# sdoira/U96-SLAM

Hardware: AMD Instinct MI355X
Metric: Mpix-disparities/s (higher is better)
Workload: dtype u8

## Files before the change

### u96-slam_amd/csrc/sbm_api.hip

```cpp
#include <stdio.h>
#include <stdlib.h>
#include <string.h>

#include <algorithm>
#include <mutex>
#include <new>

#include "sbm_handle.h"

using namespace sbm;

enum BmStage { kBmPrefilter, kBmSad, kBmBorder, kBmLr, kBmSpeckle, kBmTotal, kBmStageCount };
enum BmMark { kBmBegin, kBmPrefiltered, kBmMatched, kBmChecked, kBmEnd, kBmMarkCount };
static const char* const kBmNames[] = {"prefilter", "sad", "border", "lrcheck", "speckle", "total"};
StageTable sbm::bm_stages() { return stage_table<kBmStageCount, 0>(kBmNames); }
static_assert(kBmMarkCount == sbm_handle::kMarks, "the ring holds one event per mark");

extern "C" {

void sbm_params_default(sbm_params* p, int num_disparities, int block_size) {
  if (!p) return;
  memset(p, 0, sizeof(*p));
  p->prefilter_type = SBM_PREFILTER_XSOBEL;
  p->prefilter_size = 9;
  p->prefilter_cap = 31;
  p->block_size = block_size > 0 ? block_size : 21;
  p->min_disparity = 0;
  p->num_disparities = num_disparities > 0 ? num_disparities : 64;
  p->texture_threshold = 10;
  p->uniqueness_ratio = 15;
  p->speckle_window_size = 0;
  p->speckle_range = 0;
  p->disp12_max_diff = -1;
}

int sbm_params_validate(const sbm_params* p, int width, int height) {
  if (!p) return SBM_ERR_NULL;
  if (width <= 0 || height <= 0) return SBM_ERR_SIZE;
  if (p->prefilter_type != SBM_PREFILTER_NORMALIZED_RESPONSE && p->prefilter_type != SBM_PREFILTER_XSOBEL)
    return SBM_ERR_PREFILTER_TYPE;
  if (p->prefilter_size < 5 || p->prefilter_size > 255 || p->prefilter_size % 2 == 0) return SBM_ERR_PREFILTER_SIZE;
  if (p->prefilter_cap < 1 || p->prefilter_cap > 63) return SBM_ERR_PREFILTER_CAP;
  if (p->block_size < 5 || p->block_size > 255 || p->block_size % 2 == 0 || p->block_size >= std::min(width, height))
    return SBM_ERR_BLOCK_SIZE;
  if (p->num_disparities <= 0 || p->num_disparities % 16 != 0) return SBM_ERR_NUM_DISPARITIES;
  if (p->texture_threshold < 0) return SBM_ERR_TEXTURE;
  if (p->uniqueness_ratio < 0) return SBM_ERR_UNIQUENESS;
  return SBM_OK;
}

const char* sbm_strerror(int code) {
  switch (code) {
    case SBM_OK: return "ok";
    case SBM_ERR_NULL: return "null argument";
    case SBM_ERR_SIZE: return "bad image size or stride (all the images must have the same size)";
    case SBM_ERR_PREFILTER_TYPE: return "preFilterType must be PREFILTER_NORMALIZED_RESPONSE or PREFILTER_XSOBEL";
    case SBM_ERR_PREFILTER_SIZE: return "preFilterSize must be odd and be within 5..255";
    case SBM_ERR_PREFILTER_CAP: return "preFilterCap must be within 1..63";
    case SBM_ERR_BLOCK_SIZE: return "SADWindowSize must be odd, be within 5..255 and be not larger than image width or height";
    case SBM_ERR_NUM_DISPARITIES: return "numDisparities must be positive and divisible by 16";
    case SBM_ERR_TEXTURE: return "texture threshold must be non-negative";
    case SBM_ERR_UNIQUENESS: return "uniqueness ratio must be non-negative";
    case SBM_ERR_NO_DEVICE: return "no usable HIP device (this library has no CPU backend)";
    case SBM_ERR_HIP: return "HIP runtime error (see sbm_last_hip_error)";
    case SBM_ERR_NOMEM: return "out of memory";
    case SBM_ERR_UNSUPPORTED: return "configuration outside this build's limits";
    case SBM_ERR_BATCH: return "batch count must be positive";
    case SBM_ERR_OCC_FULL: return "occupancy map full: points were counted as overflow, not stored (see sbm_occ_overflow)";
    case SBM_ERR_VWD_FULL: return "visual-word dictionary full: the call's new words did not fit and nothing was added (see sbm_vwd_overflow)";
    default: return "unknown status";
  }
}

int sbm_version(void) { return SBM_VERSION_MAJOR * 1000 + SBM_VERSION_MINOR; }

static void free_buffers(sbm_handle* h) {
  h->each_set([](auto& s) { release_all(s); });
  release_set(h->bm); release_set(h->fp); release_set(h->fq);
  free_staging(h);
  h->sg.have_last = false;
}

static std::mutex g_pool_mu;
static constexpr int kPool = 4;
static constexpr size_t kPoolScratch = (size_t)512 << 20;
static sbm_handle* g_pool[kPool];
static int g_pool_n = 0;

static size_t scratch_bytes(sbm_handle* h) {
  size_t n = h->pin_bytes;
  h->each_set([&](auto& s) { n += bytes_held(s); });
  return n;
}

static void reset_profile(sbm_handle* h, int enabled) {
  h->profiling = enabled;
  h->calls = h->ncall = 0;
  h->instr = false;
  h->each_clock([](StageClock& c, const StageTable&) { c.reset(); });
}

static void destroy_now(sbm_handle* h);

void sbm_trim(void) {
  std::lock_guard<std::mutex> lock(g_pool_mu);
  for (int i = 0; i < g_pool_n; i++) destroy_now(g_pool[i]);
  g_pool_n = 0;
}

int sbm_create(sbm_handle** out, const sbm_params* p, int device) {
  if (!out || !p) return SBM_ERR_NULL;
  *out = nullptr;
  int ndev = 0;
  if (hipGetDeviceCount(&ndev) != hipSuccess || ndev <= 0 || device < 0 || device >= ndev) return SBM_ERR_NO_DEVICE;
  {
    std::lock_guard<std::mutex> lock(g_pool_mu);
    for (int i = 0; i < g_pool_n; i++)
      if (g_pool[i]->device == device) {
        sbm_handle* h = g_pool[i];
        g_pool[i] = g_pool[--g_pool_n];
        h->p = *p;
        h->last_hip = 0;
        h->have_last = h->sg.have_last = false;
        reset_profile(h, 0);
        *out = h;
        return SBM_OK;
      }
  }
  sbm_handle* h = new (std::nothrow) sbm_handle();
  if (!h) return SBM_ERR_NOMEM;
  memset(h, 0, sizeof(*h));
  h->p = *p;
  h->device = device;
  DeviceScope dscope(device);
  if (dscope.enter() != hipSuccess) {
    delete h;
    return SBM_ERR_NO_DEVICE;
  }
  bool ok = hipStreamCreateWithFlags(&h->stream, hipStreamNonBlocking) == hipSuccess;
  if (!ok) {
    destroy_now(h);
    return SBM_ERR_HIP;
  }
  h->ev_ok = true;
  for (int r = 0; r < sbm_handle::kRing; r++)
    for (int i = 0; i < sbm_handle::kMarks; i++) h->ev_ok &= hipEventCreate(&h->ev[r][i]) == hipSuccess;
  *out = h;
  return SBM_OK;
}

static void sync_all_streams(sbm_handle* h) {
  if (h->stream) hipStreamSynchronize(h->stream);
  if (h->stream_in) hipStreamSynchronize(h->stream_in);
  if (h->stream_out) hipStreamSynchronize(h->stream_out);
}

void sbm_destroy(sbm_handle* h) {
  if (!h) return;
  DeviceScope dscope(h->device);
  dscope.enter();
  h->fq_pending_dst = nullptr;
  h->fq_waited = h->fq_submitted;
  sync_all_streams(h);
  {
    std::lock_guard<std::mutex> lock(g_pool_mu);
    if (g_pool_n < kPool) {
      if (scratch_bytes(h) > kPoolScratch) {
        free_buffers(h);
      }
      g_pool[g_pool_n++] = h;
      return;
    }
  }
  destroy_now(h);
}

static void destroy_now(sbm_handle* h) {
  DeviceScope dscope(h->device);
  dscope.enter();
  sync_all_streams(h);
  free_buffers(h);
  h->each_clock([](StageClock& c, const StageTable&) { c.release(); });
  for (int r = 0; r < sbm_handle::kRing; r++)
    for (int i = 0; i < sbm_handle::kMarks; i++)
      if (h->ev[r][i]) hipEventDestroy(h->ev[r][i]);
  for (int i = 0; i < sbm_handle::kChunks; i++) {
    if (h->ev_in[i]) hipEventDestroy(h->ev_in[i]);
    if (h->ev_done[i]) hipEventDestroy(h->ev_done[i]);
  }
  for (int k = 0; k < 4; k++) {
    if (h->ev_fq_in[k]) hipEventDestroy(h->ev_fq_in[k]);
    if (h->ev_fq_done[k]) hipEventDestroy(h->ev_fq_done[k]);
    if (h->ev_fq_out[k]) hipEventDestroy(h->ev_fq_out[k]);
  }
  if (h->stream_in) hipStreamDestroy(h->stream_in);
  if (h->stream_out) hipStreamDestroy(h->stream_out);
  if (h->stream) hipStreamDestroy(h->stream);
  delete h;
}

int sbm_set_params(sbm_handle* h, const sbm_params* p) {
  if (!h || !p) return SBM_ERR_NULL;
  h->p = *p;
  return SBM_OK;
}

int sbm_get_params(const sbm_handle* h, sbm_params* p) {
  if (!h || !p) return SBM_ERR_NULL;
  *p = h->p;
  return SBM_OK;
}

void* sbm_stream(sbm_handle* h) { return h ? (void*)h->stream : nullptr; }
int sbm_last_hip_error(const sbm_handle* h) { return h ? h->last_hip : 0; }

int sbm_synchronize(sbm_handle* h) {
  if (!h) return SBM_ERR_NULL;
  DeviceScope dscope(h->device);
  HIPCHK(h, dscope.enter());
  HIPCHK(h, hipStreamSynchronize(h->stream));
  while (h->fq_waited != h->fq_submitted) {
    const int st = sbm_wait_oldest(h);
    if (st != SBM_OK) return st;
  }
  return SBM_OK;
}

int sbm_set_profiling(sbm_handle* h, int enabled) {
  if (!h) return SBM_ERR_NULL;
  reset_profile(h, enabled);
  return SBM_OK;
}

}

static void valid_roi(const sbm_params& p, int W, int H, int reading, int roi[4]) {
  int full[4] = {0, 0, W, H};
  const int* r1 = (p.roi1[2] > 0 && p.roi1[3] > 0) ? p.roi1 : full;
  const int* r2 = (p.roi2[2] > 0 && p.roi2[3] > 0) ? p.roi2 : full;
  const int sw2 = p.block_size / 2, maxd = p.min_disparity + p.num_disparities - 1;
  const int xmin = std::max(r1[0], r2[0] + maxd) + sw2;
  const int xmax = std::min(r1[0] + r1[2], r2[0] + r2[2] - ((reading & kReadRoiMinusMinD) ? p.min_disparity : 0)) - sw2;
  const int ymin = std::max(r1[1], r2[1]) + sw2;
  const int ymax = std::min(r1[1] + r1[3], r2[1] + r2[3]) - sw2;
  if (xmax - xmin > 0 && ymax - ymin > 0) {
    roi[0] = xmin; roi[1] = ymin; roi[2] = xmax - xmin; roi[3] = ymax - ymin;
  } else {
    roi[0] = roi[1] = roi[2] = roi[3] = 0;
  }
}

int sbm::bm_plan_geom(const sbm_params& p, int n, int width, int height, BmPlan* pl) {
  const int st = sbm_params_validate(&p, width, height);
  if (st != SBM_OK) return st;
  if (n > 32767 || height > 65535) return SBM_ERR_UNSUPPORTED;
  if (p.num_disparities > 4096) return SBM_ERR_UNSUPPORTED;
  memset(pl, 0, sizeof(*pl));
  Geom& g = pl->g;
  g.W = width; g.H = height; g.n = n;
  g.nd = p.num_disparities; g.mindisp = p.min_disparity; g.wsz = p.block_size; g.w2 = p.block_size / 2;
  g.cap = p.prefilter_cap; g.tex = p.texture_threshold; g.uniq = p.uniqueness_ratio;
  g.filtered = (p.min_disparity - 1) * 16;
  g.lofs = std::max(g.nd - 1 + g.mindisp, 0);
  g.rofs = -std::min(g.nd - 1 + g.mindisp, 0);
  g.width1 = width - g.rofs - g.nd + 1;
  g.xend = std::min(g.width1, width - g.lofs);
  g.want_cost = p.disp12_max_diff >= 0;
  g.padl = ((g.nd + 64 + 63) / 64) * 64;
  g.pitch = ((g.padl + width + 128 + 63) / 64) * 64;
  g.plane = g.pitch * height;

  int roi[4];
  g.reading = env_switch("SBM_CV_READING", 0);
  valid_roi(p, width, height, g.reading, roi);
  g.row0 = std::max(roi[1], 0); g.row1 = std::min(roi[1] + roi[3], height);
  g.col0 = std::max(std::min(roi[0], width), 0); g.col1 = std::max(std::min(roi[0] + roi[2], width), 0);
  const bool range_fits = !(g.lofs >= width || g.rofs >= width || g.width1 < 1);
  pl->any_rows = range_fits && roi[2] > 0 && roi[3] > 0 && g.row1 > g.row0;
  if (!pl->any_rows) { g.row0 = g.row1 = 0; }
  pl->in_envelope = pl->any_rows && sad_fast_supported(g);
  return SBM_OK;
}

void sbm::bm_plan_launches(const sbm_params& p, bool inplace_ok, BmPlan* pl) {
  Geom& g = pl->g;
  pl->fast = pl->in_envelope && inplace_ok;
  if (pl->fast) {
    g.cost16 = 1;
    g.pfshift = sad_fast_pfshift(g);
    const int xhi = std::min(g.W - g.lofs - 1, g.W - g.rofs - g.nd);
    const int fa = g.w2, fb = xhi - g.w2 + 1;
    const bool borders_visible = g.want_cost || g.col0 < g.lofs + fa || g.col1 > g.lofs + fb;
    pl->border = borders_visible && sad_fast_borders_in_launch(g);
    pl->wide_borders = borders_visible && !pl->border;
    pl->sad = kSadFast;
    sad_fast_plan(pl);
    if (pl->wide_borders) { pl->wide_l[0] = 0; pl->wide_l[1] = pl->f.xc0; pl->wide_r[0] = pl->f.xc1; pl->wide_r[1] = g.xend; }
  } else if (pl->any_rows) {
    const bool wide = sad_wide_supported(g) && env_switch("SBM_WIDE", 1);
    pl->sad = wide ? kSadWide : kSadGeneric;
    snprintf(pl->kernel, sizeof(pl->kernel), "%s",
             !wide ? "sad_generic_kernel" : (pl->in_envelope ? "sad_wide_kernel [in-place accumulate unavailable]" : "sad_wide_kernel"));
  }
  pl->speckle = p.speckle_range >= 0 && p.speckle_window_size > 0;
  if (pl->speckle) {
    speckle_plan(g, p.speckle_window_size, p.speckle_range, &pl->spk);
    size_t part[4];
    SpeckleScratch::bytes(g.n, g.W, g.H, part);
    for (int i = 0; i < 4; i++) pl->spk_bytes[i] = (long long)part[i];
  }
}

extern "C" {

static int ensure_scratch(sbm_handle* h, int n, int W, int H, int pitch, bool need_cost, bool need_speckle, size_t ho_bytes,
                          size_t ho_flags) {
  auto& s = h->bm;
  const bool fits = n <= s.n && W == s.W && H == s.H && pitch == s.pitch && s.pf_l.p;
  if (!fits) {
    HIPCHK(h, hipStreamSynchronize(h->stream));
    release_set(s);
    const size_t npix = (size_t)n * W * H, pfbytes = (size_t)n * pitch * H + 4096;
    HIPCHK(h, s.pf_l.grow(pfbytes, h->stream));
    HIPCHK(h, s.pf_r.grow(pfbytes, h->stream));
    HIPCHK(h, s.disp_pre.grow(npix * sizeof(int16_t), h->stream));
    HIPCHK(h, hipMemsetAsync(s.pf_l.p, 0, pfbytes, h->stream));
    HIPCHK(h, hipMemsetAsync(s.pf_r.p, 0, pfbytes, h->stream));
    s.n = n; s.W = W; s.H = H; s.pitch = pitch;
  }
  const size_t npix = (size_t)s.n * W * H;
  if (need_cost) HIPCHK(h, s.cost.grow(npix * sizeof(int32_t), h->stream));
  HIPCHK(h, s.lr_keys.grow(lr_keys_bytes(s.n, W, H, need_cost), h->stream));
  if (need_speckle) HIPCHK(h, s.spk.ensure(s.n, W, H, h->stream));
  if (ho_bytes) {
    const bool fresh = ho_bytes > s.handoff.bytes;
    HIPCHK(h, s.handoff.grow(ho_bytes, h->stream));
    if (fresh || ho_flags != s.ho_flags || s.ho_epoch == 0xffffffffu) {
      HIPCHK(h, hipMemsetAsync(s.handoff.p, 0, ho_flags, h->stream));
      s.ho_flags = ho_flags;
      s.ho_epoch = 0;
    }
  }
  return SBM_OK;
}

static inline void mark(sbm_handle* h, BmMark i) {
  if (h->instr) hipEventRecord(h->ev[h->calls % sbm_handle::kRing][i], h->stream);
}

static void collect_profile(sbm_handle* h) {
  unsigned nrec = std::min<unsigned>(h->calls, sbm_handle::kRing), first = 0;
  if (h->profiling == 1 && h->calls > 0) { first = (h->calls - 1) % sbm_handle::kRing; nrec = 1; }
  static const BmStage kStage[kBmMarkCount - 1] = {kBmPrefilter, kBmSad, kBmLr, kBmSpeckle};
  float acc[kBmMarkCount - 1] = {}, tot = 0.f;
  for (unsigned r = first; r < first + nrec; r++) {
    for (int i = 0; i < kBmMarkCount - 1; i++) {
      float ms = 0.f;
      if (hipEventElapsedTime(&ms, h->ev[r][i], h->ev[r][i + 1]) == hipSuccess) acc[i] += ms;
    }
    float ms = 0.f;
    if (hipEventElapsedTime(&ms, h->ev[r][kBmBegin], h->ev[r][kBmEnd]) == hipSuccess) tot += ms;
  }
  const float inv = nrec ? 1.f / nrec : 0.f;
  for (int i = 0; i < kBmMarkCount - 1; i++) h->bm.clock.ms[kStage[i]] = acc[i] * inv;
  h->bm.clock.ms[kBmTotal] = tot * inv;
}

int sbm_compute_device(sbm_handle* h, int n, const void* d_left, const void* d_right, int width, int height,
                       void* d_disp, int sync) {
  if (!h || !d_left || !d_right || !d_disp) return SBM_ERR_NULL;
  if (n <= 0) return SBM_ERR_BATCH;
  const sbm_params& p = h->p;
  BmPlan pl;
  const int st = bm_plan_geom(p, n, width, height, &pl);
  if (st != SBM_OK) return st;
  DeviceScope dscope(h->device);
  HIPCHK(h, dscope.enter());
  bool inplace = false;
  if (pl.in_envelope) HIPCHK(h, mqsad_inplace_ok(h->stream, &inplace));
  bm_plan_launches(p, inplace, &pl);
  const Geom& g = pl.g;
  size_t ho_flags = 0;
  const size_t ho_bytes = sad_fast_handoff_bytes(pl, &ho_flags);
  const int st2 = ensure_scratch(h, n, width, height, g.pitch, g.want_cost, pl.speckle, ho_bytes, ho_flags);
  if (st2 != SBM_OK) return st2;
  h->last = g; h->have_last = true;
  h->bm.ho_links = 0;
  if (pl.any_rows) snprintf(h->last_kernel, sizeof(h->last_kernel), "%s", pl.kernel);

  const uint8_t* dl = (const uint8_t*)d_left;
  const uint8_t* dr = (const uint8_t*)d_right;
  uint8_t *pf_l = h->bm.pf_l.as<uint8_t>(), *pf_r = h->bm.pf_r.as<uint8_t>();
  int16_t* disp_pre = h->bm.disp_pre.as<int16_t>();
  int32_t* cost = h->bm.cost.as<int32_t>();
  int16_t* out = (int16_t*)d_disp;

  h->instr = h->profiling && h->ev_ok && (h->profiling != 3 || (h->ncall & 3u) == 0);
  mark(h, kBmBegin);
  if (pl.any_rows) {
    if (p.prefilter_type == SBM_PREFILTER_XSOBEL) {
      HIPCHK(h, launch_prefilter(dl, dr, pf_l, pf_r, g, h->stream));
    } else {
      HIPCHK(h, h->bm.vsum.grow((size_t)2 * h->bm.n * width * height * sizeof(uint16_t), h->stream));
      HIPCHK(h, launch_prefilter_norm(dl, dr, pf_l, pf_r, h->bm.vsum.as<uint16_t>(), g, p.prefilter_size, h->stream));
    }
  }
  mark(h, kBmPrefiltered);
  if (pl.sad == kSadFast) {
    h->bm.ho_slots = (size_t)(pl.f.nseg - 1) * g.n * pl.f.strips;
    HIPCHK(h, launch_sad_fast(pf_l, pf_r, disp_pre, cost, pl, ho_bytes ? h->bm.handoff.p : nullptr, ho_bytes ? ++h->bm.ho_epoch : 0u,
                              &h->bm.ho_links, h->stream));
    if (pl.wide_borders) {
      HIPCHK(h, launch_sad_wide(pf_l, pf_r, disp_pre, cost, g, pl.wide_l[0], pl.wide_l[1], h->stream));
      HIPCHK(h, launch_sad_wide(pf_l, pf_r, disp_pre, cost, g, pl.wide_r[0], pl.wide_r[1], h->stream));
    }
  } else if (pl.sad == kSadWide) {
    HIPCHK(h, launch_sad_wide(pf_l, pf_r, disp_pre, cost, g, 0, g.xend, h->stream));
  } else if (pl.sad == kSadGeneric) {
    HIPCHK(h, launch_sad_generic(pf_l, pf_r, disp_pre, cost, g, 0, g.xend, h->stream));
  }
  mark(h, kBmMatched);
  HIPCHK(h, launch_lrcheck(disp_pre, cost, out, h->bm.lr_keys.as<unsigned long long>(), g, p.disp12_max_diff, h->stream));
  mark(h, kBmChecked);
  if (pl.speckle) HIPCHK(h, launch_speckle(out, h->bm.spk, g, pl.spk, p.speckle_window_size, h->stream));
  mark(h, kBmEnd);
  if (h->instr) h->calls++;
  h->ncall++;
  if (sync || h->profiling == 1) HIPCHK(h, hipStreamSynchronize(h->stream));
  return SBM_OK;
}

int sbm_debug_plan(const sbm_params* p, int n, int width, int height, int inplace_ok, void* out, size_t out_bytes) {
  if (!p || !out) return SBM_ERR_NULL;
  if (out_bytes != sizeof(BmPlan)) return SBM_ERR_SIZE;
  if (n <= 0) return SBM_ERR_BATCH;
  BmPlan pl;
  const int st = bm_plan(*p, n, width, height, inplace_ok != 0, &pl);
  if (st == SBM_OK) memcpy(out, &pl, sizeof(pl));
  return st;
}

int sbm_rect_map_device(sbm_handle* h, const sbm_rect_cam* cam, int width, int height, void* d_map, int sync) {
  if (!h || !cam || !d_map) return SBM_ERR_NULL;
  if (width <= 0 || height <= 0 || width > 32767 || height > 32767) return SBM_ERR_SIZE;
  DeviceScope dscope(h->device);
  HIPCHK(h, dscope.enter());
  HIPCHK(h, launch_rect_map(*cam, width, height, (int16_t*)d_map, h->stream));
  if (sync) HIPCHK(h, hipStreamSynchronize(h->stream));
  return SBM_OK;
}

int sbm_rect_remap_device(sbm_handle* h, int n, const void* d_src, const void* d_map, int width, int height, void* d_dst,
                          int sync) {
  if (!h || !d_src || !d_map || !d_dst) return SBM_ERR_NULL;
  if (n <= 0) return SBM_ERR_BATCH;
  if (width <= 0 || height <= 0 || width > 32767 || height > 32767) return SBM_ERR_SIZE;
  if (((size_t)width * height + 1023) / 1024 > 65535) return SBM_ERR_UNSUPPORTED;
  DeviceScope dscope(h->device);
  HIPCHK(h, dscope.enter());
  HIPCHK(h, launch_rect_remap((const uint8_t*)d_src, (const int16_t*)d_map, (uint8_t*)d_dst, n, width, height, h->stream));
  if (sync) HIPCHK(h, hipStreamSynchronize(h->stream));
  return SBM_OK;
}

int sbm_prefilter_device(sbm_handle* h, int n, const void* d_src, int width, int height, int flavour, int cap,
                         void* d_dst, int sync) {
  if (!h || !d_src || !d_dst) return SBM_ERR_NULL;
  if (n <= 0) return SBM_ERR_BATCH;
  if (width <= 0 || height <= 0) return SBM_ERR_SIZE;
  if (flavour != SBM_PREFILTER_FLAVOUR_CV && flavour != SBM_PREFILTER_FLAVOUR_RTL) return SBM_ERR_PREFILTER_TYPE;
  if (flavour == SBM_PREFILTER_FLAVOUR_CV && (cap < 1 || cap > 63)) return SBM_ERR_PREFILTER_CAP;
  if (n > 65534 || height > 65535 * 4) return SBM_ERR_UNSUPPORTED;
  DeviceScope dscope(h->device);
  HIPCHK(h, dscope.enter());
  HIPCHK(h, launch_prefilter_dense((const uint8_t*)d_src, (uint8_t*)d_dst, n, width, height,
                                   flavour == SBM_PREFILTER_FLAVOUR_RTL, cap, h->stream));
  if (sync) HIPCHK(h, hipStreamSynchronize(h->stream));
  return SBM_OK;
}

int sbm_disparity_to_float_device(sbm_handle* h, int n, const void* d_disp, int width, int height, void* d_out, int sync) {
  if (!h || !d_disp || !d_out) return SBM_ERR_NULL;
  if (n <= 0) return SBM_ERR_BATCH;
  if (width <= 0 || height <= 0) return SBM_ERR_SIZE;
  DeviceScope dscope(h->device);
  HIPCHK(h, dscope.enter());
  HIPCHK(h, launch_disp_to_float((const int16_t*)d_disp, (float*)d_out, (size_t)n * width * height, h->stream));
  if (sync) HIPCHK(h, hipStreamSynchronize(h->stream));
  return SBM_OK;
}

int sbm_decimate_device(sbm_handle* h, int n, const void* d_disp, int width, int height, int scale, void* d_out, int sync) {
  if (!h || !d_disp || !d_out) return SBM_ERR_NULL;
  if (n <= 0) return SBM_ERR_BATCH;
  if (width <= 0 || height <= 0 || scale <= 0) return SBM_ERR_SIZE;
  DeviceScope dscope(h->device);
  HIPCHK(h, dscope.enter());
  HIPCHK(h, launch_decimate((const int16_t*)d_disp, (int16_t*)d_out, n, width, height, scale, h->stream));
  if (sync) HIPCHK(h, hipStreamSynchronize(h->stream));
  return SBM_OK;
}

int sbm_reproject_device(sbm_handle* h, int n, const void* d_disp, int width, int height, int scale,
                         const sbm_stereo_model* model, int apply_local, void* d_xyz, int sync) {
  if (!h || !d_disp || !d_xyz || !model) return SBM_ERR_NULL;
  if (n <= 0) return SBM_ERR_BATCH;
  if (width <= 0 || height <= 0 || scale <= 0) return SBM_ERR_SIZE;
  DeviceScope dscope(h->device);
  HIPCHK(h, dscope.enter());
  HIPCHK(h, launch_reproject((const int16_t*)d_disp, (float*)d_xyz, n, width, height, scale, *model, apply_local, h->stream));
  if (sync) HIPCHK(h, hipStreamSynchronize(h->stream));
  return SBM_OK;
}

int sbm_keypoints3d_device(sbm_handle* h, const void* d_disp, int width, int height, const void* d_kpts, int nk,
                           const sbm_stereo_model* model, float min_depth, float max_depth, void* d_xyz, int sync) {
  if (!h || !d_disp || !model || (nk > 0 && (!d_kpts || !d_xyz))) return SBM_ERR_NULL;
  if (width <= 0 || height <= 0 || nk < 0) return SBM_ERR_SIZE;
  DeviceScope dscope(h->device);
  HIPCHK(h, dscope.enter());
  HIPCHK(h, launch_keypoints3d((const int16_t*)d_disp, (const float*)d_kpts, (float*)d_xyz, width, height, nk, *model,
                               min_depth, max_depth, h->stream));
  if (sync) HIPCHK(h, hipStreamSynchronize(h->stream));
  return SBM_OK;
}

int sbm_get_profile(sbm_handle* h, const char* name, float* ms) {
  if (!h || !name || !ms) return SBM_ERR_NULL;
  DeviceScope dscope(h->device);
  HIPCHK(h, dscope.enter());
  HIPCHK(h, hipStreamSynchronize(h->stream));
  if (h->profiling && h->ev_ok) collect_profile(h);
  const float* t = nullptr;
  h->each_clock([&](StageClock& c, const StageTable& tab) {
    for (int i = 0; i < tab.nstage; i++)
      if (!strcmp(name, tab.names[i])) t = &c.ms[i];
  });
  if (!t) return SBM_ERR_UNSUPPORTED;
  *ms = *t;
  return SBM_OK;
}

int sbm_last_kernel_name(sbm_handle* h, char* dst, size_t dst_bytes) {
  if (!h || !dst || dst_bytes == 0) return SBM_ERR_NULL;
  snprintf(dst, dst_bytes, "%s", h->last_kernel);
  return SBM_OK;
}

int sbm_debug_fetch(sbm_handle* h, int which, void* dst, size_t dst_bytes) {
  if (!h || !dst) return SBM_ERR_NULL;
  if (which >= 4 && which <= 6) return sgbm_debug_fetch(h, which, dst, dst_bytes);
  if (!h->have_last) return SBM_ERR_UNSUPPORTED;
  const Geom& g = h->last;
  DeviceScope dscope(h->device);
  HIPCHK(h, dscope.enter());
  HIPCHK(h, hipStreamSynchronize(h->stream));
  const size_t npix = (size_t)g.n * g.W * g.H;
  if (which == 0 || which == 1) {
    if (dst_bytes < npix) return SBM_ERR_SIZE;
    const uint8_t* src = (which == 0 ? h->bm.pf_l : h->bm.pf_r).as<uint8_t>();
    HIPCHK(h, hipMemcpy2D(dst, g.W, src + g.padl, g.pitch, g.W, (size_t)g.n * g.H, hipMemcpyDeviceToHost));
    uint8_t* d = (uint8_t*)dst;
    for (size_t i = 0; i < npix; i++) d[i] = (uint8_t)((d[i] - kPfBias) >> g.pfshift);
    return SBM_OK;
  }
  if (which == 2) {
    if (!h->bm.cost.p) return SBM_ERR_UNSUPPORTED;
    if (dst_bytes < npix * sizeof(int32_t)) return SBM_ERR_SIZE;
    if (g.cost16) {
      uint16_t* tmp = (uint16_t*)malloc(npix * sizeof(uint16_t));
      if (!tmp) return SBM_ERR_NOMEM;
      hipError_t e = hipMemcpy(tmp, h->bm.cost.p, npix * sizeof(uint16_t), hipMemcpyDeviceToHost);
      if (e == hipSuccess)
        for (size_t i = 0; i < npix; i++) ((int32_t*)dst)[i] = tmp[i];
      free(tmp);
      HIPCHK(h, e);
      return SBM_OK;
    }
    HIPCHK(h, hipMemcpy(dst, h->bm.cost.p, npix * sizeof(int32_t), hipMemcpyDeviceToHost));
    return SBM_OK;
  }
  if (which == 3) {
    if (dst_bytes < npix * sizeof(int16_t)) return SBM_ERR_SIZE;
    HIPCHK(h, hipMemcpy(dst, h->bm.disp_pre.p, npix * sizeof(int16_t), hipMemcpyDeviceToHost));
    int16_t* d = (int16_t*)dst;
    for (int i = 0; i < g.n; i++)
      for (int y = 0; y < g.H; y++) {
        int16_t* row = d + ((size_t)i * g.H + y) * g.W;
        const bool live = y >= g.row0 && y < g.row1;
        for (int x = 0; x < g.W; x++)
          if (!live || x < g.lofs || x >= g.lofs + g.xend) row[x] = (int16_t)g.filtered;
      }
    return SBM_OK;
  }
  if (which == 7) {
    if (dst_bytes < 2 * sizeof(int32_t)) return SBM_ERR_SIZE;
    int32_t* d = (int32_t*)dst;
    d[0] = 0;
    d[1] = (int32_t)h->bm.ho_links;
    if (!h->bm.ho_links) return SBM_OK;
    const size_t slots = h->bm.ho_slots;
    uint32_t* tmp = (uint32_t*)malloc(slots * sizeof(uint32_t));
    if (!tmp) return SBM_ERR_NOMEM;
    const hipError_t e = hipMemcpy(tmp, h->bm.handoff.as<uint32_t>() + slots, slots * sizeof(uint32_t), hipMemcpyDeviceToHost);
    if (e == hipSuccess)
      for (size_t i = 0; i < slots; i++) d[0] += tmp[i] == h->bm.ho_epoch;
    free(tmp);
    HIPCHK(h, e);
    return SBM_OK;
  }
  return SBM_ERR_UNSUPPORTED;
}

}
```

### u96-slam_amd/csrc/sbm_sad_fast.hip

```cpp
#include <string.h>

#include "sbm_sad_fast_kernel.h"

namespace sbm {

__global__ void __launch_bounds__(256) mqsad_inplace_selftest_kernel(unsigned* bad) {
  unsigned long long st = (unsigned long long)(blockIdx.x * 256 + threadIdx.x) * 0x9E3779B97F4A7C15ull + 88172645463325252ull;
  auto rnd = [&]() { st ^= st << 13; st ^= st >> 7; st ^= st << 17; return st; };
  unsigned nbad = 0;
  for (int it = 0; it < 64; it++) {
    unsigned long long accA[4], accR[4], win[4];
    const unsigned pat = (unsigned)rnd() & ((it & 1) ? 0x00ffffffu : 0x000000ffu);
#pragma unroll
    for (int q = 0; q < 4; q++) { accA[q] = accR[q] = rnd() & 0x3fff3fff3fff3fffull; win[q] = rnd(); }
#pragma unroll
    for (int r = 0; r < 3; r++)
#pragma unroll
      for (int q = 0; q < 4; q++) {
        accR[q] = __builtin_amdgcn_mqsad_pk_u16_u8(win[(q + r) & 3], pat, accR[q]);
        asm volatile("v_mqsad_pk_u16_u8 %0, %1, %2, %0" : "+v"(accA[q]) : "v"(win[(q + r) & 3]), "v"(pat));
      }
#pragma unroll
    for (int q = 0; q < 4; q++) nbad += accA[q] != accR[q];
  }
  if (nbad) atomicAdd(bad, nbad);
  atomicAdd(bad + 1, 1u);
}

hipError_t mqsad_inplace_ok(hipStream_t s, bool* ok) {
  static const bool forced_off = env_switch("SBM_FAST_INPLACE", 1) == 0;
  static std::mutex mu;
  static signed char known[64];
  *ok = false;
  int dev = 0;
  hipError_t e = hipGetDevice(&dev);
  if (e != hipSuccess || forced_off || dev < 0 || dev >= 64) return e;
  std::lock_guard<std::mutex> lock(mu);
  if (!known[dev]) {
    unsigned* d = nullptr;
    if ((e = hipMalloc(&d, 8)) != hipSuccess) return e;
    bool pass = true;
    const unsigned grids[3] = {256u, 1024u, 2048u};
    for (int k = 0; k < 3 && pass && e == hipSuccess; k++) {
      unsigned h[2] = {1u, 0u};
      e = hipMemsetAsync(d, 0, 8, s);
      if (e == hipSuccess) {
        hipLaunchKernelGGL(mqsad_inplace_selftest_kernel, dim3(grids[k]), dim3(256), 0, s, d);
        e = hipGetLastError();
      }
      if (e == hipSuccess) e = hipMemcpyAsync(h, d, 8, hipMemcpyDeviceToHost, s);
      if (e == hipSuccess) e = hipStreamSynchronize(s);
      pass = h[0] == 0u && h[1] == grids[k] * 256u;
    }
    const hipError_t ef = hipFree(d);
    if (e == hipSuccess) e = ef;
    if (e != hipSuccess) return e;
    known[dev] = pass ? 1 : -1;
  }
  *ok = known[dev] > 0;
  return hipSuccess;
}

int sad_fast_pfshift(const Geom& g) {
  static const int env = env_switch("SBM_FAST_PFSHIFT", 2);
  if (env <= 0 || !sad_fast_supported(g)) return 0;
  const long maxs = (long)g.wsz * g.wsz * 2 * g.cap;
  const int sh = std::min(env, g.wsz <= 15 ? 2 : 1);
  const long f = 1L << sh;
  if (f * 2 * g.cap + 1 > 255) return 0;
  if (f * maxs + (f - 1) > 65535) return 0;
  if (2 * (f * (maxs * g.uniq / 100 + 1)) >= 65535) return 0;
  if ((long)g.tex * f > 0x3fffffff) return 0;
  return sh == (g.wsz <= 15 ? 2 : 1) ? sh : 0;
}

bool sad_fast_borders_in_launch(const Geom& g) { return g.nd <= 256; }

bool sad_fast_supported(const Geom& g) {
  if (g.wsz < 5 || g.wsz > 31) return false;
  if (g.nd > kFastNdMax) return false;
  const long maxs = (long)g.wsz * g.wsz * 2 * g.cap;
  if (maxs > 65534) return false;
  if (2 * (maxs * g.uniq / 100 + 1) >= 65535) return false;
  if (g.row0 < g.w2 || g.row1 > g.H - g.w2 || g.row1 <= g.row0) return false;
  if ((long)g.plane * 4 >= (1L << 31)) return false;
  const int xhi = std::min(g.W - g.lofs - 1, g.W - g.rofs - g.nd);
  if (xhi - g.w2 + 1 <= g.w2) return false;
  return true;
}

static hipError_t sad_fast_dispatch(BmPlan& pl, const FastArgs* a, hipStream_t s) {
  switch (pl.g.wsz) {
    case 15: return launch_nd<5, 3>(pl, a, s);
    case 21: return launch_nd<7, 3>(pl, a, s);
    default: return launch_sad_fast_pw1(pl, a, s);
  }
}

static int fast_handoff_mode() { return std::max(0, std::min(2, env_switch("SBM_FAST_HANDOFF", 1))); }

static int fast_slots(int nd) { return nd <= 64 ? 4096 : 3072; }

constexpr double kFirstRoundStep = 0.10, kFirstRoundSpan = 0.40;

static int fast_segment_order(int nseg, long per_seg, int slots, int nd, unsigned char* at) {
  for (int k = 0; k < 64; k++) at[k] = (unsigned char)k;
  if (fast_handoff_mode() != 1 || nd > 128) return nseg;
  const long D = (slots + per_seg - 1) / per_seg + 1;
  if (D >= nseg) return nseg;
  int base = 0;
  for (int r = 0; r < (int)D; r++)
    for (int p = r; p < nseg; p += (int)D) at[p] = (unsigned char)base++;
  return (int)D;
}

void sad_fast_plan(BmPlan* pl) {
  const Geom& g = pl->g;
  FastPlan& a = pl->f;
  const int xhi = std::min(g.W - g.lofs - 1, g.W - g.rofs - g.nd);
  a.xc0 = g.w2; a.xc1 = xhi - g.w2 + 1;
  const int pw = g.wsz % 3 == 0 ? 3 : 1;
  const int nv = 64 - (g.wsz - pw);
  const int cs3_env = env_switch("SBM_FAST_CS3", 1);
  const int ncols = a.xc1 - a.xc0;
  const int nv3 = 64 - (g.wsz / 3 - 1);
  int triples = 0;
  if (pw == 3 && cs3_env) {
    triples = ncols / (3 * nv3);
    if (ncols - triples * 3 * nv3 > 2 * nv) triples++;
  }
  a.strips3 = 3 * triples;
  const int rem = std::max(0, ncols - triples * 3 * nv3);
  const int strips = a.strips3 + (rem + nv - 1) / nv;
  const int rows = g.row1 - g.row0;
  const int round1 = g.nd <= 256 ? 1536 : (g.nd <= 384 ? 1024 : 768);
  constexpr double kSegC = 0.196;
  const int slots_i = g.nd <= 64 ? 4096 : (g.nd <= 128 ? 3072 : round1);
  int nseg = 1;
  {
    const double prime = 0.2 * (g.wsz - 1);
    const double slots = slots_i;
    nseg = (int)(std::sqrt(kSegC * slots * rows / ((double)strips * g.n * prime)) + 0.5);
    nseg = std::max(1, std::min(nseg, std::max(1, rows / g.wsz)));
  }
  constexpr int kSmallRows = 8;
  constexpr long kFill = 5000;
  const int maxseg = std::max(nseg, std::min(64, rows / kSmallRows));
  const long per_seg = (long)strips * g.n;
  if (per_seg * maxseg * (g.nd > 128 ? (g.nd + 127) / 128 : 1) < 1800) {
    nseg = std::max(nseg, (int)std::min<long>(maxseg, 1023 / per_seg));
  } else {
    const int nseg1 = nseg;
    while (per_seg * nseg < kFill && nseg < maxseg) nseg++;
    if (g.nd > 128 && per_seg * nseg > round1 && 2 * per_seg * nseg < 3 * round1) nseg = std::max(nseg1, (int)((long)round1 * 1450 / 1536 / per_seg));
  }
  nseg = std::min(nseg, 64);
  int ns = 0;
  a.segrow[0] = g.row0;
  if (nseg < 3) {
    const int seg = (rows + nseg - 1) / nseg;
    for (int y = g.row0; y < g.row1; y += seg) a.segrow[++ns] = std::min(y + seg, g.row1);
  } else {
    unsigned char at[64];
    const int stride = fast_segment_order(nseg, per_seg, slots_i, g.nd, at);
    const int first_round = stride - 1;
    int len[64];
    {
      const double step = first_round > 1 ? std::min(kFirstRoundStep, kFirstRoundSpan / (first_round - 1)) : 0.0;
      double wgt[64], sum = 0;
      for (int p = 0; p < nseg; p++) {
        wgt[p] = p < nseg - 3 ? 1.0 : (p == nseg - 3 ? 0.75 : (p == nseg - 2 ? 0.5 : 0.25));
        if (stride < nseg && p < first_round) wgt[p] = std::min(wgt[p], 1.0 - step * (first_round - 1 - p));
        sum += wgt[p];
      }
      const double unit = rows / sum;
      double acc = 0;
      int y0 = 0;
      for (int p = 0; p < nseg; p++) {
        acc += wgt[p] * unit;
        const int y1 = p == nseg - 1 ? rows : std::min(rows, (int)(acc + 0.5));
        len[p] = y1 - y0;
        y0 = y1;
      }
    }
    int np = 0;
    for (int p = 0; p < nseg; p++)
      if (len[p] > 0) len[np++] = len[p];
    fast_segment_order(np, per_seg, slots_i, g.nd, at);
    int seglen[64];
    for (int p = 0; p < np; p++) seglen[at[p]] = len[p];
    for (int k = 0; k < np; k++) a.segrow[k + 1] = a.segrow[k] + seglen[k];
    ns = np;
  }
  nseg = ns;
  a.strips = strips; a.nseg = nseg;
  {
    const long maxs = (long)g.wsz * g.wsz * 2 * g.cap;
    a.uniq_plain = 8 * ((maxs * g.uniq / 100 + 1) << g.pfshift) <= 65535;
  }
  a.split = (long)strips * nseg * g.n < 1024;
  sad_fast_dispatch(*pl, nullptr, nullptr);
}

static unsigned long long fast_handoff_links(const BmPlan& pl, unsigned char* at) {
  const FastPlan& f = pl.f;
  const int mode = fast_handoff_mode();
  const int stride = fast_segment_order(f.nseg, (long)f.strips * pl.g.n, fast_slots(pl.g.nd), pl.g.nd, at);
  if (mode == 0 || f.NWAVES != 1 || !f.exact || f.nseg < 2) return 0;
  unsigned long long links = 0;
  for (int p = mode == 2 ? 1 : stride; p < f.nseg; p++) links |= 1ull << at[p];
  return links;
}

constexpr size_t kHandoffMaxBytes = (size_t)1 << 30;
size_t sad_fast_handoff_bytes(const BmPlan& pl, size_t* flag_bytes) {
  unsigned char at[64];
  *flag_bytes = 0;
  if (!pl.fast || !fast_handoff_links(pl, at)) return 0;
  const size_t slots = (size_t)(pl.f.nseg - 1) * pl.g.n * pl.f.strips;
  const size_t fb = (2 * slots * sizeof(u32) + 255) & ~(size_t)255;
  const size_t bytes = fb + slots * ((size_t)(pl.f.NDW / 4) * 512 + 256);
  if (bytes > kHandoffMaxBytes) return 0;
  *flag_bytes = fb;
  return bytes;
}

hipError_t launch_sad_fast(const uint8_t* pf_l, const uint8_t* pf_r, int16_t* disp, int32_t* cost, BmPlan& pl, void* handoff,
                           unsigned epoch, long* links, hipStream_t s) {
  const Geom& g = pl.g;
  const FastPlan& f = pl.f;
  FastArgs a;
  a.pf_l = pf_l; a.pf_r = pf_r; a.disp = disp; a.cost = g.want_cost ? reinterpret_cast<uint16_t*>(cost) : nullptr;
  a.W = g.W; a.H = g.H; a.pitch = g.pitch; a.padl = g.padl; a.plane = g.plane;
  a.nd = g.nd; a.mindisp = g.mindisp; a.lofs = g.lofs; a.rofs = g.rofs; a.tex = g.tex << g.pfshift; a.uniq = g.uniq;
  a.filtered = g.filtered; a.capb = (g.cap << g.pfshift) + kPfBias; a.pfshift = g.pfshift;
  a.row0 = g.row0; a.row1 = g.row1;
  static_assert(sizeof(a.segrow) == sizeof(f.segrow), "");
  memcpy(a.segrow, f.segrow, sizeof(a.segrow));
  a.strips = f.strips; a.nseg = f.nseg; a.npairs = g.n; a.strips3 = f.strips3; a.uniq_plain = f.uniq_plain;
  a.xc0 = f.xc0; a.xc1 = f.xc1;
  a.bord = f.bord; a.bnw = f.bnw; a.bseg = f.bseg; a.nbseg = f.nbseg;
  a.ho_link = fast_handoff_links(pl, a.segat);
  if (!handoff) a.ho_link = 0;
  a.ho = static_cast<u32*>(handoff); a.ho_epoch = epoch;
  a.segbase = 0; a.grid = f.grid;
  const long per_seg = (long)f.strips * g.n;
  *links = (long)__builtin_popcountll(a.ho_link) * per_seg;
  if (fast_handoff_mode() != 2 || !a.ho_link) return sad_fast_dispatch(pl, &a, s);
  for (int k = 0; k < f.nseg; k++) {
    a.segbase = k;
    a.grid = (int)per_seg + (k == 0 ? f.bord * f.nbseg : 0);
    if (k == 1) a.bord = 0;
    const hipError_t e = sad_fast_dispatch(pl, &a, s);
    if (e != hipSuccess) return e;
  }
  return hipSuccess;
}

}
```

### u96-slam_amd/csrc/sbm_sad_fast_strip.h

```cpp
#pragma once
#include "sbm_sad_fast_core.h"

namespace sbm {

template <int NDW, int NWAVES, int NTERM, int PW, bool EXACT_ND, int CS>
__device__ __forceinline__ void sad_fast_strip_dma(const FastArgs& a, unsigned char* __restrict__ const b0c, unsigned char* __restrict__ const b1c,
                                                   unsigned char* __restrict__ const xl1c,
                                                   u32* __restrict__ const xkey,
                                                   const int cbase, const int segi, const int pair, const int strip) {
  using L = FastLds<NDW, NTERM, PW, CS>;
  using D = DmaLds<NDW, NWAVES, NTERM, PW, CS>;
  using P = HPlan<NTERM, PW>;
  typedef __attribute__((address_space(3))) void* lds_vptr;
  constexpr int NQ = NDW / 4;
  constexpr int NR = NDW / 2;
  constexpr int NSLOT = L::NSLOT;
  constexpr int NIT = NSLOT / 64;
  constexpr int WSZ = PW * NTERM, W2 = WSZ / 2;
  constexpr int KS = L::KS;
  constexpr int NV = 64 - KS * (NTERM - 1);
  constexpr int XCH = D::XCH, XS = L::XS;
  constexpr bool HANDOFF = FastHandoff<NDW, NWAVES, EXACT_ND>::ON;

  const int lane = threadIdx.x & 63;
  const int wv = NWAVES > 1 ? __builtin_amdgcn_readfirstlane(threadIdx.x >> 6) : 0;
  const int d0 = wv * NDW;
  const int ndl = EXACT_ND ? NDW : a.nd - d0;
  const int c = cbase + CS * lane;
  const int xc = c + W2;
  const bool produces = lane < NV && xc >= a.xc0 && xc < a.xc1;
  const int ys = a.segrow[segi];
  const int ye = a.segrow[segi + 1];
  const uint8_t* pl = a.pf_l + (size_t)pair * a.plane + a.padl + a.lofs + cbase;
  const uint8_t* pr = a.pf_r + (size_t)pair * a.plane + a.padl + a.rofs + cbase + d0;
  uint2* const xacc = reinterpret_cast<uint2*>(xkey + 2 * NWAVES * 64);
  const unsigned lane_u = (unsigned)lane;
  const __amdgpu_buffer_rsrc_t rs_l = __builtin_amdgcn_make_buffer_rsrc(const_cast<uint8_t*>(pl), 0, 0x7fffffff, 0x00020000);
  const __amdgpu_buffer_rsrc_t rs_r = __builtin_amdgcn_make_buffer_rsrc(const_cast<uint8_t*>(pr), 0, 0x7fffffff, 0x00020000);
  uint4* const b0 = reinterpret_cast<uint4*>(b0c);
  uint4* const b1 = reinterpret_cast<uint4*>(b1c);
  uint4* const xq0 = b0;
  uint4* const xq1 = reinterpret_cast<uint4*>(xl1c);
  typedef u32x4 __attribute__((may_alias)) u32x4a;
  auto xt_of = [](uint4* const xq) { return reinterpret_cast<u32*>(xq + (XCH / 2) * XS); };
  const u32 capw = (u32)a.capb * 0x01010101u;

  u64 VB[NQ];
  {
    const u32 unit = (lane_u / (unsigned)KS) % (unsigned)NTERM == 0u ? FastTag<WSZ>::tag_unit(a.pfshift) : 0u;
#pragma unroll
    for (int q = 0; q < NQ; q++) {
      const u32 tq = (u32)((2 * q) / (NR / FastTag<WSZ>::NGRP)) * unit;
      VB[q] = __builtin_bit_cast(u64, make_uint2(tq, tq));
    }
  }
  u32 Vt = 0;

  auto pat_of = [](uint4* const buf) { return reinterpret_cast<u32*>(reinterpret_cast<unsigned char*>(buf) + D::PAT_OFS); };
  auto stage = [&](const int y, uint4* const buf) {
    const int rowoff = __builtin_amdgcn_readfirstlane(y * a.pitch);
#pragma unroll
    for (int it = 0; it < NIT; it++)
      __builtin_amdgcn_raw_ptr_buffer_load_lds(rs_r, (lds_vptr)(reinterpret_cast<u32*>(buf) + 64 * it), 4, (int)lane_u, rowoff + 64 * it, 0, 0);
    __builtin_amdgcn_raw_ptr_buffer_load_lds(rs_l, (lds_vptr)pat_of(buf), 4, (int)(CS * lane_u), rowoff, 0, 0);
  };
  auto landed = [] {
    __builtin_amdgcn_s_waitcnt(0);
    __builtin_amdgcn_fence(__ATOMIC_ACQUIRE, "wavefront");
    __builtin_amdgcn_wave_barrier();
  };
  auto reads_done = [] {
    __builtin_amdgcn_s_waitcnt(0xc07f);
    __builtin_amdgcn_wave_barrier();
  };
  auto published = [] {
    __builtin_amdgcn_fence(__ATOMIC_RELEASE, "wavefront");
    __builtin_amdgcn_wave_barrier();
  };
  auto apply = [&](uint4* const buf, const bool leave) {
    constexpr u32 PMASK = PW == 3 ? 0x00ffffffu : 0x000000ffu;
    const u32 pat = pat_of(buf)[lane] & PMASK;
    const u32 tv = __builtin_amdgcn_sad_u8(pat | (capw & ~PMASK), capw, 0u);
    auto quad = [&](const int q, const u32 lo, const u32 hi) {
      const u64 win = ((u64)hi << 32) | lo;
      if (!leave) {
        asm("v_mqsad_pk_u16_u8 %0, %1, %2, %0" : "+v"(VB[q]) : "v"(win), "v"(pat));
      } else {
        const uint2 tt = __builtin_bit_cast(uint2, __builtin_amdgcn_mqsad_pk_u16_u8(win, pat, 0ull));
        uint2 vb = __builtin_bit_cast(uint2, VB[q]);
        vb.x -= tt.x;
        vb.y -= tt.y;
        asm("" : "+v"(vb.x), "+v"(vb.y));
        VB[q] = __builtin_bit_cast(u64, vb);
      }
    };
    {
      const u32* const win4 = reinterpret_cast<const u32*>(buf) + CS * lane;
      if constexpr (EXACT_ND) {
  #pragma unroll
        for (int q0 = 0; q0 < NQ; q0 += 16) {
          u32 lo[16], hi[16];
  #pragma unroll
          for (int qq = 0; qq < 16 && q0 + qq < NQ; qq++) { lo[qq] = win4[4 * (q0 + qq)]; hi[qq] = win4[4 * (q0 + qq) + 4]; }
  #pragma unroll
          for (int qq = 0; qq < 16 && q0 + qq < NQ; qq++) quad(q0 + qq, lo[qq], hi[qq]);
        }
      } else {
  #pragma unroll
        for (int g = 0; g < NQ / 4; g++) {
          if (16 * g < ndl) {
            u32 lo[4], hi[4];
  #pragma unroll
            for (int k = 0; k < 4; k++) { lo[k] = win4[4 * (4 * g + k)]; hi[k] = win4[4 * (4 * g + k) + 4]; }
  #pragma unroll
            for (int k = 0; k < 4; k++) quad(4 * g + k, lo[k], hi[k]);
          }
        }
      }
    }
    Vt = leave ? Vt - tv : Vt + tv;
  };

  const size_t ho_slots = HANDOFF ? (size_t)(a.nseg - 1) * a.npairs * a.strips : 0;
  const size_t ho_mine = HANDOFF ? ((size_t)segi * a.npairs + pair) * a.strips + strip : 0;
  auto ho_rsrc = [&](const size_t slot) {
    unsigned char* const p = reinterpret_cast<unsigned char*>(a.ho) + ((2 * ho_slots * sizeof(u32) + 255) & ~(size_t)255) + slot * FastHandoff<NDW, NWAVES, EXACT_ND>::SLOT_B;
    return __builtin_amdgcn_make_buffer_rsrc(p, 0, FastHandoff<NDW, NWAVES, EXACT_ND>::SLOT_B, 0x00020000);
  };
  bool take = false;
  if constexpr (HANDOFF) {
    if ((a.ho_link >> segi) & 1) {
      const size_t from = ho_mine - (size_t)a.npairs * a.strips;
      take = __builtin_amdgcn_readfirstlane(__hip_atomic_load(a.ho + from, __ATOMIC_RELAXED, __HIP_MEMORY_SCOPE_AGENT)) == a.ho_epoch;
      if (take) {
        __builtin_amdgcn_fence(__ATOMIC_ACQUIRE, "agent");
        const __amdgpu_buffer_rsrc_t rs_h = ho_rsrc(from);
#pragma unroll
        for (int q = 0; q < NQ; q++) VB[q] = __builtin_bit_cast(u64, __builtin_amdgcn_raw_buffer_load_b64(rs_h, (int)(8 * lane_u), 512 * q, kHandoffAux));
        Vt = __builtin_amdgcn_raw_buffer_load_b32(rs_h, (int)(4 * lane_u), 512 * NQ, kHandoffAux);
        if (lane == 0) a.ho[ho_slots + from] = a.ho_epoch;
        stage(ys + W2, b0);
      }
    }
  }
  if (!take) {
    stage(ys - W2, b0);
    for (int i = 0; i < 2 * W2; i += 2) {
      landed();
      stage(ys - W2 + i + 1, b1);
      apply(b0, false);
      landed();
      stage(ys - W2 + i + 2, b0);
      apply(b1, false);
    }
  }
  const __amdgpu_buffer_rsrc_t rs_d = __builtin_amdgcn_make_buffer_rsrc(a.disp + (size_t)pair * a.W * a.H, 0, 0x7fffffff, 0x00020000);
  const __amdgpu_buffer_rsrc_t rs_c = __builtin_amdgcn_make_buffer_rsrc(a.cost + (size_t)pair * a.W * a.H, 0, 0x7fffffff, 0x00020000);
  const int ocol_u = __builtin_amdgcn_readfirstlane(2 * (a.lofs + cbase + W2));
  u32 res_prev = 0xffff0000u;
  auto flush = [&](const int yrow) {
    if (produces && (NWAVES == 1 || (yrow % NWAVES) == wv)) {
      const int orow_prev = __builtin_amdgcn_readfirstlane(2 * yrow * a.W) + ocol_u;
      u32 l3 = CS * lane_u;
      asm volatile("" : "+v"(l3));
      const int ocol = (int)(2 * l3);
      if (a.cost) __builtin_amdgcn_raw_buffer_store_b16((short)(res_prev >> 16), rs_c, ocol, orow_prev, 0);
      __builtin_amdgcn_raw_buffer_store_b16((short)res_prev, rs_d, ocol, orow_prev, 0);
    }
  };
  for (int y = ys; y < ye; y++) {
    landed();
    if (y > ys) {
      flush(y - 1);
      apply(b1, true);
    }
    reads_done();
    stage(y - W2, b1);
    apply(b0, false);

    __builtin_amdgcn_s_setprio(kFastPrioExchange);
    u32 S[NR];
    unsigned long long tex_ok = 0;
    u32 lx = lane_u;
    asm volatile("" : "+v"(lx));
    auto add4 = [](u32 (&acc)[4], const uint4 r) { acc[0] += r.x; acc[1] += r.y; acc[2] += r.z; acc[3] += r.w; };
#pragma unroll
    for (int q0 = 0; q0 < NQ; q0 += XCH) {
      const bool tex_now = q0 == 0;
      if (!EXACT_ND && 4 * q0 >= ndl) {
#pragma unroll
        for (int j = 2 * q0; j < 2 * (q0 + XCH); j++) S[j] = 0xffffffffu;
        continue;
      }
      u32 A[XCH / 2][4];
      u32 tA = Vt;
#pragma unroll
      for (int e = 0; e < XCH / 2; e++) {
        const uint2 v0 = __builtin_bit_cast(uint2, VB[q0 + 2 * e]), v1 = __builtin_bit_cast(uint2, VB[q0 + 2 * e + 1]);
        A[e][0] = v0.x; A[e][1] = v0.y; A[e][2] = v1.x; A[e][3] = v1.y;
        xq0[e * XS + lane] = make_uint4(v0.x, v0.y, v1.x, v1.y);
      }
      if (tex_now) xt_of(xq0)[lane] = Vt;
      published();
      if constexpr (P::S1 > 1) {
#pragma unroll
        for (int e = 0; e < XCH / 2; e++)
#pragma unroll
          for (int k = 1; k < P::S1; k++) add4(A[e], xq0[e * XS + lx + KS * k]);
        if (tex_now)
#pragma unroll
          for (int k = 1; k < P::S1; k++) tA += xt_of(xq0)[lx + KS * k];
        if constexpr (P::PUB1) {
#pragma unroll
          for (int e = 0; e < XCH / 2; e++) {
            if constexpr (HANDOFF) *reinterpret_cast<u32x4a*>(xq1 + e * XS + lane) = (u32x4){A[e][0], A[e][1], A[e][2], A[e][3]};
            else xq1[e * XS + lane] = make_uint4(A[e][0], A[e][1], A[e][2], A[e][3]);
          }
          if (tex_now) xt_of(xq1)[lane] = tA;
          published();
        }
      }
      {
        constexpr int OV = P::NTT * P::S1;
#pragma unroll
        for (int e = 0; e < XCH / 2; e++) {
#pragma unroll
          for (int t = 1; t < P::NTT; t++) {
            if constexpr (HANDOFF) {
              const u32x4 r = *reinterpret_cast<const u32x4a*>(xq1 + e * XS + lx + KS * P::S1 * t);
              add4(A[e], make_uint4(r.x, r.y, r.z, r.w));
            } else {
              add4(A[e], xq1[e * XS + lx + KS * P::S1 * t]);
            }
          }
#pragma unroll
          for (int v = (P::NTT > 0 ? 0 : 1); v < P::NVV; v++) add4(A[e], xq0[e * XS + lx + KS * (OV + v)]);
        }
        if (tex_now) {
#pragma unroll
          for (int t = 1; t < P::NTT; t++) tA += xt_of(xq1)[lx + KS * P::S1 * t];
#pragma unroll
          for (int v = (P::NTT > 0 ? 0 : 1); v < P::NVV; v++) tA += xt_of(xq0)[lx + KS * (OV + v)];
          tex_ok = __ballot((int)tA >= a.tex);
        }
      }
#pragma unroll
      for (int e = 0; e < XCH / 2; e++)
#pragma unroll
        for (int i = 0; i < 4; i++) S[2 * (q0 + 2 * e) + i] = A[e][i];
      __builtin_amdgcn_wave_barrier();
    }
    reads_done();
    stage(min(y + 1 + W2, a.H - 1), b0);
    __builtin_amdgcn_s_setprio(0);

    u32 best = fast_first_min<NR, WSZ>(S, a.pfshift);
    best += (u32)d0;
    const int par = y & 1, mpar = par * NWAVES * 64;
    if constexpr (NWAVES > 1) {
      xkey[mpar + wv * 64 + lane] = best;
      __syncthreads();
#pragma unroll
      for (int w = 0; w < NWAVES; w++) best = min(best, xkey[mpar + w * 64 + lane]);
    }
    const int minsad = (int)(best >> 16), mind = (int)(best & 0xffffu);

    u32 acc = 0, T = 0;
    if (a.uniq > 0) {
      T = fast_uniq_threshold(minsad, a.uniq, a.pfshift);
      acc = fast_deficits<NR, WSZ>(S, T, a.uniq_plain, a.pfshift);
    }

    const int in_ = mind > 0 ? mind - 1 : 1;
    const int ip_ = mind < a.nd - 1 ? mind + 1 : a.nd - 2;
    const int ln = min(max(in_ - d0, 0), NDW - 1), lp = min(max(ip_ - d0, 0), NDW - 1);
    u32 X0;
    {
      u32 X[NQ];
      const u32 lnp = (u32)ln | ((u32)lp << 16);
      fast_neighbours_quads<NQ>(S, lnp, X);
      X0 = fast_neighbours_tree<NQ>(X, lnp) & ~(((1u << a.pfshift) - 1u) * 0x00010001u);
    }
    int nn = (int)(X0 & 0xffffu), pp = (int)(X0 >> 16);
    u32 acc_lo = acc & 0xffffu, acc_hi = acc >> 16;
    bool mine = true;
    if constexpr (NWAVES > 1) {
      xacc[mpar + wv * 64 + lane] = make_uint2(acc, X0);
      __syncthreads();
      mine = (y % NWAVES) == wv;
      if (mine) {
        acc_lo = acc_hi = 0;
#pragma unroll
        for (int w = 0; w < NWAVES; w++) {
          const u32 aw = xacc[mpar + w * 64 + lane].x;
          acc_lo += aw & 0xffffu;
          acc_hi += aw >> 16;
        }
        nn = (int)(xacc[mpar + (in_ / NDW) * 64 + lane].y & 0xffffu);
        pp = (int)(xacc[mpar + (ip_ / NDW) * 64 + lane].y >> 16);
      }
    }

    bool ok = __builtin_amdgcn_inverse_ballot_w64(tex_ok);
    if (a.uniq > 0) ok = ok && fast_unique(acc_lo, acc_hi, T, minsad, mind, nn, pp, a.nd);
    if (mine && produces) {
      int out = a.filtered, cst = -1;
      if (ok) {
        out = fast_subpixel(nn, pp, minsad, mind, a.nd, a.mindisp);
        if (a.cost) cst = minsad >> a.pfshift;
      }
      res_prev = ((u32)out & 0xffffu) | ((u32)cst << 16);
    }
  }
  flush(ye - 1);
  if constexpr (HANDOFF) {
    if (segi + 1 < a.nseg && ((a.ho_link >> (segi + 1)) & 1)) {
      landed();
      apply(b1, true);
      const __amdgpu_buffer_rsrc_t rs_h = ho_rsrc(ho_mine);
#pragma unroll
      for (int q = 0; q < NQ; q++) __builtin_amdgcn_raw_buffer_store_b64(__builtin_bit_cast(u32x2, VB[q]), rs_h, (int)(8 * lane_u), 512 * q, kHandoffAux);
      __builtin_amdgcn_raw_buffer_store_b32(Vt, rs_h, (int)(4 * lane_u), 512 * NQ, kHandoffAux);
      asm volatile("s_waitcnt vmcnt(0)" ::: "memory");
      if (lane == 0) __hip_atomic_store(a.ho + ho_mine, a.ho_epoch, __ATOMIC_RELAXED, __HIP_MEMORY_SCOPE_AGENT);
    }
  }
}

}
```

Before: 4.373 million.

## Plan more row segments with compact handoff slots for linked segments only

```diff
diff --git a/u96-slam_amd/csrc/sbm_api.hip b/u96-slam_amd/csrc/sbm_api.hip
--- a/u96-slam_amd/csrc/sbm_api.hip
+++ b/u96-slam_amd/csrc/sbm_api.hip
@@ -407,9 +407,9 @@
   }
   mark(h, kBmPrefiltered);
   if (pl.sad == kSadFast) {
-    h->bm.ho_slots = (size_t)(pl.f.nseg - 1) * g.n * pl.f.strips;
     HIPCHK(h, launch_sad_fast(pf_l, pf_r, disp_pre, cost, pl, ho_bytes ? h->bm.handoff.p : nullptr, ho_bytes ? ++h->bm.ho_epoch : 0u,
                               &h->bm.ho_links, h->stream));
+    h->bm.ho_slots = (size_t)h->bm.ho_links;
     if (pl.wide_borders) {
       HIPCHK(h, launch_sad_wide(pf_l, pf_r, disp_pre, cost, g, pl.wide_l[0], pl.wide_l[1], h->stream));
       HIPCHK(h, launch_sad_wide(pf_l, pf_r, disp_pre, cost, g, pl.wide_r[0], pl.wide_r[1], h->stream));
@@ -438,6 +438,18 @@
   const int st = bm_plan(*p, n, width, height, inplace_ok != 0, &pl);
   if (st == SBM_OK) memcpy(out, &pl, sizeof(pl));
   return st;
+}
+
+int sbm_debug_handoff_bytes(const sbm_params* p, int n, int width, int height, int inplace_ok, uint64_t* out) {
+  if (!p || !out) return SBM_ERR_NULL;
+  if (n <= 0) return SBM_ERR_BATCH;
+  BmPlan pl;
+  const int st = bm_plan(*p, n, width, height, inplace_ok != 0, &pl);
+  if (st != SBM_OK) return st;
+  size_t flags = 0;
+  out[0] = sad_fast_handoff_bytes(pl, &flags);
+  out[1] = flags;
+  return SBM_OK;
 }
 
 int sbm_rect_map_device(sbm_handle* h, const sbm_rect_cam* cam, int width, int height, void* d_map, int sync) {
diff --git a/u96-slam_amd/csrc/sbm_sad_fast.hip b/u96-slam_amd/csrc/sbm_sad_fast.hip
--- a/u96-slam_amd/csrc/sbm_sad_fast.hip
+++ b/u96-slam_amd/csrc/sbm_sad_fast.hip
@@ -114,6 +114,42 @@
   return (int)D;
 }
 
+constexpr size_t kHandoffMaxBytes = (size_t)1 << 30;
+static size_t fast_handoff_size(long linked, long per_seg, int ndw, size_t* flag_bytes) {
+  const size_t slots = (size_t)linked * per_seg;
+  *flag_bytes = (2 * slots * sizeof(u32) + 255) & ~(size_t)255;
+  return *flag_bytes + slots * ((size_t)(ndw / 4) * 512 + 256);
+}
+
+constexpr double kHandoffRows = 0.7, kSegCLinked = 0.12;
+static int fast_linked_plan(const Geom& g, int rows, long per_seg, int slots, int nseg, int maxseg, int* len) {
+  if (nseg < 3 || (g.nd != 32 && g.nd != 64 && g.nd != 128)) return 0;
+  unsigned char at[64];
+  const int D = fast_segment_order(nseg, per_seg, slots, g.nd, at);
+  if (D >= nseg) return 0;
+  int n = (int)(std::sqrt(kSegCLinked * slots * rows / ((double)per_seg * kHandoffRows)) + 0.5);
+  n = std::max(nseg, std::min(n, std::min(maxseg, 64)));
+  size_t fb;
+  while (n > nseg && fast_handoff_size(n - D, per_seg, g.nd, &fb) > kHandoffMaxBytes) n--;
+  if (fast_handoff_size(n - D, per_seg, g.nd, &fb) > kHandoffMaxBytes) return 0;
+  const int fr = D - 1;
+  const double step = fr > 1 ? std::min(kFirstRoundStep, kFirstRoundSpan / (fr - 1)) : 0.0;
+  double wgt[64], sum = 0;
+  for (int p = 0; p < n; p++) {
+    wgt[p] = p < fr ? 1.0 - step * (fr - 1 - p) : (double)(n - p) / (n - fr);
+    sum += wgt[p];
+  }
+  const double unit = rows / sum;
+  int left = rows;
+  for (int p = 0; p < n; p++) {
+    len[p] = (int)(wgt[p] * unit);
+    left -= len[p];
+  }
+  for (int p = fr; p < n && left > 0; p++, left--) len[p]++;
+  for (int p = fr - 1; p >= 0 && left > 0; p--, left--) len[p]++;
+  return n;
+}
+
 void sad_fast_plan(BmPlan* pl) {
   const Geom& g = pl->g;
   FastPlan& a = pl->f;
@@ -155,6 +191,8 @@
     if (g.nd > 128 && per_seg * nseg > round1 && 2 * per_seg * nseg < 3 * round1) nseg = std::max(nseg1, (int)((long)round1 * 1450 / 1536 / per_seg));
   }
   nseg = std::min(nseg, 64);
+  int len[64];
+  const int linked = fast_linked_plan(g, rows, per_seg, slots_i, nseg, maxseg, len);
   int ns = 0;
   a.segrow[0] = g.row0;
   if (nseg < 3) {
@@ -164,8 +202,9 @@
     unsigned char at[64];
     const int stride = fast_segment_order(nseg, per_seg, slots_i, g.nd, at);
     const int first_round = stride - 1;
-    int len[64];
-    {
+    if (linked) {
+      nseg = linked;
+    } else {
       const double step = first_round > 1 ? std::min(kFirstRoundStep, kFirstRoundSpan / (first_round - 1)) : 0.0;
       double wgt[64], sum = 0;
       for (int p = 0; p < nseg; p++) {
@@ -212,14 +251,14 @@
   return links;
 }
 
-constexpr size_t kHandoffMaxBytes = (size_t)1 << 30;
 size_t sad_fast_handoff_bytes(const BmPlan& pl, size_t* flag_bytes) {
   unsigned char at[64];
   *flag_bytes = 0;
-  if (!pl.fast || !fast_handoff_links(pl, at)) return 0;
-  const size_t slots = (size_t)(pl.f.nseg - 1) * pl.g.n * pl.f.strips;
-  const size_t fb = (2 * slots * sizeof(u32) + 255) & ~(size_t)255;
-  const size_t bytes = fb + slots * ((size_t)(pl.f.NDW / 4) * 512 + 256);
+  if (!pl.fast) return 0;
+  const unsigned long long links = fast_handoff_links(pl, at);
+  if (!links) return 0;
+  size_t fb = 0;
+  const size_t bytes = fast_handoff_size(__builtin_popcountll(links), (long)pl.g.n * pl.f.strips, pl.f.NDW, &fb);
   if (bytes > kHandoffMaxBytes) return 0;
   *flag_bytes = fb;
   return bytes;
diff --git a/u96-slam_amd/csrc/sbm_sad_fast_strip.h b/u96-slam_amd/csrc/sbm_sad_fast_strip.h
--- a/u96-slam_amd/csrc/sbm_sad_fast_strip.h
+++ b/u96-slam_amd/csrc/sbm_sad_fast_strip.h
@@ -121,8 +121,9 @@
     Vt = leave ? Vt - tv : Vt + tv;
   };
 
-  const size_t ho_slots = HANDOFF ? (size_t)(a.nseg - 1) * a.npairs * a.strips : 0;
-  const size_t ho_mine = HANDOFF ? ((size_t)segi * a.npairs + pair) * a.strips + strip : 0;
+  const size_t ho_set = HANDOFF ? (size_t)a.npairs * a.strips : 0;
+  const size_t ho_slots = HANDOFF ? (size_t)__builtin_popcountll(a.ho_link) * ho_set : 0;
+  auto ho_slot = [&](const int k) { return (size_t)__builtin_popcountll(a.ho_link & ((1ull << k) - 1)) * ho_set + (size_t)pair * a.strips + strip; };
   auto ho_rsrc = [&](const size_t slot) {
     unsigned char* const p = reinterpret_cast<unsigned char*>(a.ho) + ((2 * ho_slots * sizeof(u32) + 255) & ~(size_t)255) + slot * FastHandoff<NDW, NWAVES, EXACT_ND>::SLOT_B;
     return __builtin_amdgcn_make_buffer_rsrc(p, 0, FastHandoff<NDW, NWAVES, EXACT_ND>::SLOT_B, 0x00020000);
@@ -130,7 +131,7 @@
   bool take = false;
   if constexpr (HANDOFF) {
     if ((a.ho_link >> segi) & 1) {
-      const size_t from = ho_mine - (size_t)a.npairs * a.strips;
+      const size_t from = ho_slot(segi);
       take = __builtin_amdgcn_readfirstlane(__hip_atomic_load(a.ho + from, __ATOMIC_RELAXED, __HIP_MEMORY_SCOPE_AGENT)) == a.ho_epoch;
       if (take) {
         __builtin_amdgcn_fence(__ATOMIC_ACQUIRE, "agent");
@@ -317,6 +318,7 @@
     if (segi + 1 < a.nseg && ((a.ho_link >> (segi + 1)) & 1)) {
       landed();
       apply(b1, true);
+      const size_t ho_mine = ho_slot(segi + 1);
       const __amdgpu_buffer_rsrc_t rs_h = ho_rsrc(ho_mine);
 #pragma unroll
       for (int q = 0; q < NQ; q++) __builtin_amdgcn_raw_buffer_store_b64(__builtin_bit_cast(u32x2, VB[q]), rs_h, (int)(8 * lane_u), 512 * q, kHandoffAux);
```

Result: faster. 4.441 million, median of 6 (+1.6%).
